# dcy0577/Enhancing-3D-Point-Cloud-Segmentation-Using-Multi-Modal-Fusion-with-2D-Images

Hardware: AMD Instinct MI355X
Metric: input points/s through MV-KPConv KPFCNN forward+backward (pyramid + fusion + fwd + bwd + SGD) (higher is better)
Workload: dtype f32; 1 GPU; early_fusion_kpfcnn5_sphere19k_x1_per_gpu; views=3, parallelism=dp1, execution=hipGraph[net|chain|enc2d(x2 every 2nd step)+fa], ranks=1, input_lookahead_batches=2, capacity_overflow=False

## Files before the change

### enhancing-3d-point-cloud-segmentation-using-multi-modal-fusion-with-2d-images_amd/_lib.py

```python
import ctypes as C
import os
import re

_HERE = os.path.dirname(os.path.abspath(__file__))
LIB_PATH = os.path.join(_HERE, "libmvkpconv.so")
HEADER_PATH = os.path.join(_HERE, "..", "include", "mvkpconv.h")
SCENE_HEADER_PATH = os.path.join(_HERE, "..", "include", "mvkpconv_scene.h")
TRAIN_HEADER_PATH = os.path.join(_HERE, "..", "include", "mvkpconv_train.h")
SPHERE_HEADER_PATH = os.path.join(_HERE, "..", "include", "mvkpconv_sphere.h")

CTYPES = {"int": C.c_int, "int32_t": C.c_int32, "int64_t": C.c_int64, "float": C.c_float, "double": C.c_double,
          "const char*": C.c_char_p}
_SCALARS = frozenset(t for t in CTYPES if not t.endswith("*"))
_POINTEES = _SCALARS | {"void", "char", "uint8_t", "uint16_t"}
_INTEGER = r"-?(?:0[xX][0-9a-fA-F]+|0|[1-9][0-9]*)"
_DIRECTIVE = re.compile(r"\s*#\s*(?:include\s*<[\w./]+>|ifdef\s+__cplusplus|ifndef\s+\w+_H|endif"
                        r"|define\s+(\w+)(?:\s+(%s))?)\s*" % _INTEGER)
_STRUCT = re.compile(r"typedef\s+struct(?:\s+\w+)?\s*\{([^{}]*)\}\s*(mvk_\w+)\s*;")
_FUNCTION = re.compile(r"([\w\s*]+?)\b(mvk_\w+)\s*\(([^(){};]*)\)\s*;")


def parse_header(text):
    functions, structs, constants = {}, {}, {}

# ... 101 lines not shown
    raise ValueError("mvkpconv_scene.h: it may declare neither a struct nor a name of mvkpconv.h")
_SCENE_PROTOTYPES = _bind(SCENE_FUNCTIONS, {})[1]

TRAIN_FUNCTIONS, _train_structs, TRAIN_CONSTANTS = parse_header(_read_header(TRAIN_HEADER_PATH, "mvkpconv_train.h"))
if (_train_structs or TRAIN_FUNCTIONS.keys() & (FUNCTIONS.keys() | SCENE_FUNCTIONS.keys())
        or TRAIN_CONSTANTS.keys() & (CONSTANTS.keys() | SCENE_CONSTANTS.keys())):
    raise ValueError("mvkpconv_train.h: it may declare neither a struct nor a name of the other two headers")
_TRAIN_PROTOTYPES = _bind(TRAIN_FUNCTIONS, {})[1]

SPHERE_FUNCTIONS, _sphere_structs, SPHERE_CONSTANTS = parse_header(_read_header(SPHERE_HEADER_PATH, "mvkpconv_sphere.h"))
if (_sphere_structs
        or SPHERE_FUNCTIONS.keys() & (FUNCTIONS.keys() | SCENE_FUNCTIONS.keys() | TRAIN_FUNCTIONS.keys())
        or SPHERE_CONSTANTS.keys() & (CONSTANTS.keys() | SCENE_CONSTANTS.keys() | TRAIN_CONSTANTS.keys())):
    raise ValueError("mvkpconv_sphere.h: it may declare neither a struct nor a name of the other three headers")
_SPHERE_PROTOTYPES = _bind(SPHERE_FUNCTIONS, {})[1]
BnFwdProblem, BnBwdProblem = _CLASSES["mvk_bn_fwd_problem"], _CLASSES["mvk_bn_bwd_problem"]
BnFinish, ATransform = _CLASSES["mvk_bn_finish"], _CLASSES["mvk_a_transform"]
RevList, RegLayer = _CLASSES["mvk_rev_list"], _CLASSES["mvk_reg_layer"]

_lib = None
_owner_pid = None

FORK_MESSAGE = ("the MV-KPConv HIP library was initialised in process %d and is being called from its forked child %d: "
                "a HIP context does not survive fork(). Start DataLoader workers with multiprocessing_context='spawn', "
                "or let the workers emit only stacked points / lengths and build the pyramid "
                "(datasets.common.segmentation_inputs_sphere) in the main process -- see INTEGRATION.md")


def _check_process():
    pid = os.getpid()
# ... 5 lines not shown
            raise RuntimeError(FORK_MESSAGE % (os.getppid(), pid))
    except (ImportError, AttributeError):
        pass


def lib():
    global _lib, _owner_pid
    _check_process()
    if _lib is None:
        if not os.path.exists(LIB_PATH):
            raise RuntimeError(
                "libmvkpconv.so is not built (%s). Run `python __graft_entry__.py build` -- there is "
                "no CPU fallback for the MV-KPConv hot path." % LIB_PATH)
        l = C.CDLL(LIB_PATH)
        for name, (res, args) in list(_PROTOTYPES.items()) + list(_SCENE_PROTOTYPES.items()) + list(_TRAIN_PROTOTYPES.items()) \
                + list(_SPHERE_PROTOTYPES.items()):
            fn = getattr(l, name)
            fn.restype = res
            fn.argtypes = args
        if l.mvk_abi_version() != ABI_VERSION:
            raise RuntimeError("libmvkpconv.so ABI %d != expected %d; rebuild" % (l.mvk_abi_version(), ABI_VERSION))
        _lib = l
        _owner_pid = os.getpid()
    return _lib


def check(rc):
    if rc != 0:
        raise RuntimeError(lib().mvk_last_error().decode("utf-8", "replace"))
```

### enhancing-3d-point-cloud-segmentation-using-multi-modal-fusion-with-2d-images_amd/build.py

```python
import os
import subprocess
import sys

HERE = os.path.dirname(os.path.abspath(__file__))
CSRC = os.path.join(HERE, "csrc")
OUT = os.path.join(HERE, "libmvkpconv.so")
ARCH = "gfx950"

SOURCES = [
    ("error.cpp", []),
    ("kpconv.hip", []),
    ("gemm.hip", []),
    ("gemm32s.hip", []),
    ("pool.hip", []),
    ("bn.hip", []),
    ("optim.hip", []),
    ("deform.hip", []),
    ("loss.hip", []),
    ("batchpad.hip", []),
    ("revlist.hip", []),
    ("subsample.hip", ["-ffp-contract=off"]),
    ("neighbors.hip", ["-ffp-contract=off"]),
    ("fusion.hip", ["-ffp-contract=off"]),
    ("vote.hip", ["-ffp-contract=off"]),
    ("pn2.hip", ["-ffp-contract=off"]),
    ("chunk.hip", ["-ffp-contract=off"]),
    ("pn2_ordered.hip", ["-ffp-contract=off"]),
    ("pn2_mlp.hip", ["-ffp-contract=off"]),
    ("pn2_rows.hip", ["-ffp-contract=off"]),
    ("scene_inputs.hip", ["-ffp-contract=off"]),
    ("train_inputs.hip", ["-ffp-contract=off"]),
    ("sphere_inputs.hip", ["-ffp-contract=off"]),
]
# ... 6 lines not shown
    return "hipcc"


def _stale(target, deps):
    if not os.path.exists(target):
        return True
    t = os.path.getmtime(target)
    return any(os.path.getmtime(d) > t for d in deps if os.path.exists(d))


def build_library(force=False, verbose=False):
    hipcc = _hipcc()
    common = [os.path.join(CSRC, "common.h"), os.path.join(CSRC, "blockscan.h"), os.path.join(CSRC, "compact.h"),
              os.path.join(CSRC, "pn2_rows.h"), os.path.join(CSRC, "unproject.h"), os.path.join(CSRC, "select_frames.h"),
              os.path.join(CSRC, "knn_core.h"), os.path.join(HERE, "..", "include", "mvkpconv_sphere.h"),
              os.path.join(HERE, "..", "include", "mvkpconv.h"), os.path.join(HERE, "..", "include", "mvkpconv_scene.h"),
              os.path.join(HERE, "..", "include", "mvkpconv_train.h"),
              os.path.join(HERE, "..", "include", "mvk_prime_list.h"), os.path.abspath(__file__)]
    objs, jobs = [], []
    for src, extra in SOURCES:
        sp = os.path.join(CSRC, src)
        if not os.path.exists(sp):
            raise FileNotFoundError(sp)
        obj = os.path.join(CSRC, os.path.splitext(src)[0] + ".o")
        if force or _stale(obj, [sp] + common):
            cmd = [hipcc, "--offload-arch=" + ARCH, "-O3", "-std=c++17", "-fPIC", "-c", sp, "-o", obj] + extra
            if src.endswith(".cpp"):
                cmd = [hipcc, "-O2", "-std=c++17", "-fPIC", "-c", sp, "-o", obj]
            jobs.append(cmd)
        objs.append(obj)
# ... 21 lines not shown
```

### enhancing-3d-point-cloud-segmentation-using-multi-modal-fusion-with-2d-images_amd/dropin/models/architectures.py

```python
import numpy as np
import torch
import torch.nn as nn

try:
    from .blocks import KPConv, UnaryBlock, NearestUpsampleBlock, block_decider
    from .._native import ops as _ops
except ImportError:
    from models.blocks import KPConv, UnaryBlock, NearestUpsampleBlock, block_decider
    from _native import ops as _ops


def p2p_fitting_regularizer(net):
    total = 0
    deform = [m for m in net.modules() if isinstance(m, KPConv) and m.deformable]
    if deform and all(m.min_d2.is_cuda for m in deform):
        term = _ops.deform_regularizer_all([(m.min_d2, m.deformed_KP, m.KP_extent, net.repulse_extent,
                                             net.deform_fitting_power, _ops.row_count_for(m.min_d2.shape[0]))
                                            for m in deform])
        return term if term is not None else total
    for m in deform:
        rows = m.min_d2.shape[0]
        n_valid = _ops.row_count_for(rows)
        if n_valid is None:
            mask, denom = None, float(rows)
# ... 85 lines not shown
        idx = labels.long().clamp(-1, lut.numel() - 2) + 1
        return lut[idx].to(labels.dtype)

    def _label_table(self, device, dtype=torch.int64):
        key = "_target_lut" if dtype == torch.int64 else "_target_lut32"
        lut = getattr(self, key, None)
        if lut is None or lut.device != device:
            top = int(max(self.valid_labels)) if len(self.valid_labels) else 0
            table = np.full(top + 3, -1, dtype=np.int64)
            for i, c in enumerate(self.valid_labels):
                table[int(c) + 1] = i
            lut = torch.from_numpy(table).to(device=device, dtype=dtype)
            setattr(self, key, lut)
        return lut

    def loss(self, outputs, labels):
        if outputs.is_cuda and outputs.dtype == torch.float32:
            self.output_loss = _ops.cross_entropy_lut(outputs, labels, self._label_table(outputs.device, torch.int32),
                                                      self.criterion.weight)
        else:
            target = self._targets(labels)
            outputs = torch.transpose(outputs, 0, 1).unsqueeze(0)
            self.output_loss = self.criterion(outputs, target.unsqueeze(0))
        if self.deform_fitting_mode == 'point2point':
            self.reg_loss = p2p_fitting_regularizer(self)
        elif self.deform_fitting_mode == 'point2plane':
            raise ValueError('point2plane fitting mode not implemented yet.')
        else:
            raise ValueError('Unknown fitting mode: ' + self.deform_fitting_mode)
        if isinstance(self.reg_loss, (int, float)) and self.reg_loss == 0:
            return self.output_loss
        return self.output_loss + self.reg_loss
# ... 56 lines not shown
    def __init__(self, config, lbl_values, ign_lbls):
        super(KPFCNN, self).__init__()
        self.K = config.num_kernel_points
        self.C = len(lbl_values) - len(ign_lbls)
        (self.encoder_blocks, self.encoder_skips, self.encoder_skip_dims,
         in_dim, out_dim, layer, r) = build_encoder(config, config.in_features_dim)
        self.decoder_blocks, self.decoder_concats, out_dim = build_decoder(
            config, in_dim, out_dim, layer, r, self.encoder_skip_dims)
        self.head_mlp = UnaryBlock(out_dim, config.first_features_dim, False, 0)
        self.head_softmax = UnaryBlock(config.first_features_dim, self.C, False, 0)
        self._init_losses(config, lbl_values, ign_lbls)

    def forward(self, batch, config):
        x = batch.features.detach()
        x = run_encoder_decoder(self, x, batch)
        return self.head_softmax(self.head_mlp(x, batch), batch)
```

### enhancing-3d-point-cloud-segmentation-using-multi-modal-fusion-with-2d-images_amd/dropin/models/architectures_sphere.py

```python
import torch
import torch.nn as nn

try:
    from .architectures import (p2p_fitting_regularizer, build_encoder, build_decoder, run_encoder_decoder,
                                _SegmentationLossMixin)
    from .blocks import UnaryBlock
    from .fusion_common import build_2d_branch, lift_2d_features
except ImportError:
    from models.architectures import (p2p_fitting_regularizer, build_encoder, build_decoder,
                                      run_encoder_decoder, _SegmentationLossMixin)
    from models.blocks import UnaryBlock
    from models.fusion_common import build_2d_branch, lift_2d_features


class KPFCNN_featureAggre(_SegmentationLossMixin, nn.Module):
    fa_output_detached = True

    def __init__(self, config, lbl_values, ign_lbls):
        super(KPFCNN_featureAggre, self).__init__()
        self.K = config.num_kernel_points
        self.C = len(lbl_values) - len(ign_lbls)
        (self.encoder_blocks, self.encoder_skips, self.encoder_skip_dims,
         in_dim, out_dim, layer, r) = build_encoder(config, config.in_features_dim)
        self.decoder_blocks, self.decoder_concats, out_dim = build_decoder(
            config, in_dim, out_dim, layer, r, self.encoder_skip_dims)
        self.head_mlp = UnaryBlock(out_dim, config.first_features_dim, False, 0)
        self.head_softmax = UnaryBlock(config.first_features_dim, self.C, False, 0)
        self._init_losses(config, lbl_values, ign_lbls)
        build_2d_branch(self, config)

    def forward(self, batch, config):
        stacked = getattr(batch, 'stacked_features', None)
        if stacked is None:
            feature_2d3d = lift_2d_features(self, batch)
            stacked = torch.cat((batch.feature_3d, feature_2d3d), dim=1)
        x = stacked.detach()
        x = run_encoder_decoder(self, x, batch)
        return self.head_softmax(self.head_mlp(x, batch), batch)
```

### enhancing-3d-point-cloud-segmentation-using-multi-modal-fusion-with-2d-images_amd/dropin/models/architectures_sphere_late_fusion.py

```python
import torch
import torch.nn as nn

try:
    from .architectures import (p2p_fitting_regularizer, build_encoder, build_decoder, run_encoder_decoder,
                                _SegmentationLossMixin)
    from .blocks import UnaryBlock
    from .fusion_common import build_2d_branch, lift_2d_features
except ImportError:
    from models.architectures import (p2p_fitting_regularizer, build_encoder, build_decoder,
                                      run_encoder_decoder, _SegmentationLossMixin)
    from models.blocks import UnaryBlock
    from models.fusion_common import build_2d_branch, lift_2d_features


class KPFCNN_featureAggre(_SegmentationLossMixin, nn.Module):

    def __init__(self, config, lbl_values, ign_lbls):
        super(KPFCNN_featureAggre, self).__init__()
        self.K = config.num_kernel_points
        self.C = len(lbl_values) - len(ign_lbls)
        (self.encoder_blocks, self.encoder_skips, self.encoder_skip_dims,
         in_dim, out_dim, layer, r) = build_encoder(config, config.in_features_dim)
        self.decoder_blocks, self.decoder_concats, out_dim = build_decoder(
            config, in_dim, out_dim, layer, r, self.encoder_skip_dims)
        self.transform_mlp = UnaryBlock(out_dim, 64, False, 0)
        self.head_mlp = UnaryBlock(out_dim, config.first_features_dim, False, 0)
        self.head_softmax = UnaryBlock(config.first_features_dim, self.C, False, 0)
        self._init_losses(config, lbl_values, ign_lbls)
        build_2d_branch(self, config)

    def forward(self, batch, config):
        feature_2d3d = lift_2d_features(self, batch)
        x = batch.feature_3d.detach()
        x = run_encoder_decoder(self, x, batch)
        x = self.transform_mlp(x, batch)
        x = torch.cat((x, feature_2d3d), dim=1)
        return self.head_softmax(self.head_mlp(x, batch), batch)
```

### enhancing-3d-point-cloud-segmentation-using-multi-modal-fusion-with-2d-images_amd/dropin/models/architectures_sphere_middle_fusion.py

```python
import torch
import torch.nn as nn

try:
    from .architectures import (p2p_fitting_regularizer, build_encoder, build_decoder, run_decoder,
                                _SegmentationLossMixin)
    from .blocks import UnaryBlock
    from .fusion_common import build_2d_branch, lift_2d_features
except ImportError:
    from models.architectures import (p2p_fitting_regularizer, build_encoder, build_decoder, run_decoder,
                                      _SegmentationLossMixin)
    from models.blocks import UnaryBlock
    from models.fusion_common import build_2d_branch, lift_2d_features


class KPFCNN_featureAggre(_SegmentationLossMixin, nn.Module):
    fa_output_detached = True

    def __init__(self, config, lbl_values, ign_lbls):
        super(KPFCNN_featureAggre, self).__init__()
        self.K = config.num_kernel_points
        self.C = len(lbl_values) - len(ign_lbls)
        (self.encoder_blocks_3d, self.encoder_skips, dims3, in3, out_dim, layer, r) = build_encoder(
            config, config.in_features_dim_3d)
        (self.encoder_blocks_2d, _, dims2, in2, _, _, _) = build_encoder(config, config.in_features_dim_2d)
# ... 11 lines not shown
        x_2d = torch.cat((ones, feature_2d3d), dim=1).detach()
        x_3d = batch.feature_3d.detach()
        skip_x = []
        for block_i, block_op in enumerate(self.encoder_blocks_3d):
            if block_i in self.encoder_skips:
                skip_x.append(x_3d)
            x_3d = block_op(x_3d, batch)
        index = 0
        for block_i, block_op in enumerate(self.encoder_blocks_2d):
            if block_i in self.encoder_skips:
                skip_x[index] = torch.cat([skip_x[index], x_2d], dim=1)
                index += 1
            x_2d = block_op(x_2d, batch)
        x = torch.mean(torch.stack([x_3d, x_2d]), 0)
        x = run_decoder(self, x, skip_x, batch)
        return self.head_softmax(self.head_mlp(x, batch), batch)
```

### enhancing-3d-point-cloud-segmentation-using-multi-modal-fusion-with-2d-images_amd/ops.py

```python
import collections
import os
import ctypes as C

import weakref

import torch

from ._lib import lib, check, CONSTANTS, SCENE_CONSTANTS, TRAIN_CONSTANTS, SPHERE_CONSTANTS

INFLUENCE = {k[len("MVK_INFL_"):].lower(): v for k, v in CONSTANTS.items() if k.startswith("MVK_INFL_")}
AGGREGATION = {k[len("MVK_AGG_"):].lower(): v for k, v in CONSTANTS.items() if k.startswith("MVK_AGG_")}


def _p(t):
    return C.c_void_p(t.data_ptr()) if t is not None else None


def _stream():
    return C.c_void_p(torch.cuda.current_stream().cuda_stream)


def _dev(*ts):
    for t in ts:
        if t is not None and not t.is_cuda:
# ... 2381 lines not shown
        d = torch.empty_like(logits)
        check(lib().mvk_xent_bwd(_p(logits), logits.shape[0], logits.shape[1], _p(labels),
                                 int(labels.dtype == torch.int64), _p(lut), lut.numel(), _p(weight), _p(out2), _p(g), _p(d),
                                 _stream()))
        return d, None, None, None


def cross_entropy_lut(logits, labels, lut, class_weight=None):
    if lut.dtype != torch.int32 or lut.dim() != 1 or lut.numel() < 3:
        raise RuntimeError("cross_entropy_lut: lut must be a 1-D int32 tensor of at least 3 entries")
    if logits.dim() != 2 or labels.dim() != 1 or labels.shape[0] != logits.shape[0]:
        raise RuntimeError("cross_entropy_lut: logits [N, C] and labels [N] expected")
    if class_weight is not None and (class_weight.dtype != torch.float32 or class_weight.numel() != logits.shape[1]):
        raise RuntimeError("cross_entropy_lut: class_weight must be float32 [C]")
    return _XentFn.apply(logits, labels, lut, None if class_weight is None else class_weight.contiguous())


_SEG_STATUS = {}


def seg_label_status(device):
    device = torch.device(device)
    key = device.index if device.index is not None else torch.cuda.current_device()
    if key not in _SEG_STATUS:
        _SEG_STATUS[key] = torch.zeros((1,), device=device, dtype=torch.int32)
    return _SEG_STATUS[key]


def seg_check_labels(device=None):
    status = seg_label_status(device if device is not None else torch.device("cuda", torch.cuda.current_device()))
# ... 781 lines not shown
```

### enhancing-3d-point-cloud-segmentation-using-multi-modal-fusion-with-2d-images_amd/step.py

```python
import os
import sys
import time

import numpy as np
import torch

from . import dp, ops, synthetic as syn

_DEV = {"on": False}
_DEV_KNOBS = ("MVK_BENCH_DIAG", "MVK_BENCH_SKIP", "MVK_BENCH_DUMMY_LAUNCHES")


def _knob(name, default=None):
    v = os.environ.get(name)
    if v is None or v == "":
        return default
    if not _DEV["on"]:
        raise RuntimeError("%s=%s is a development knob of the captured step (it changes what a step contains): pass "
                           "dev=True to GraphStep / --dev to bench.py, or unset it" % (name, v))
    return v


class GraphStep:

# ... 236 lines not shown
                else:
                    loss = torch.zeros((), device=dev)
                for h in hooks:
                    h.remove()
                if diag != "noside":
                    if not side_first and not hooks:
                        side_work()
                    join_encoder()
            return graph.replay, loss
        staged_exchange = hasattr(reducer, "cut_block")
        net.backward_cut = reducer.cut_block if staged_exchange else None
        scope = backward_scope(ops)
        with torch.cuda.graph(graph, stream=main_stream, capture_error_mode="thread_local"):
            hooks = fork_side_branches()
            ops.step_begin()
            loss = net.loss(net(static, cfg), static.labels)
            for h in hooks:
                h.remove()
            if staged_exchange:
                orig, leaves = net.cut_tensors
                with scope():
                    loss.backward(reducer.seed(loss), retain_graph=reducer.dp.deformable_below(cfg.architecture, reducer.cut_block))
                reducer.pack(0)
            else:
                backward(ops, loss)
            join_encoder()
        if not staged_exchange:
            graph_b = torch.cuda.CUDAGraph()
            with torch.cuda.graph(graph_b, stream=main_stream, pool=graph.pool(), capture_error_mode="thread_local"):
                clip_and_step(params, opt, cfg)
            grads = [p.grad for p in reducer.params if p.grad is not None]
# ... 229 lines not shown

def make_reducer(net, cfg, params, world):
    cut = dp.cut_block_of_layer(cfg.architecture, 2) if os.environ.get("MVK_DP_OVERLAP", "1") == "1" else None
    if cut is None or not hasattr(net, "encoder_blocks"):
        return dp.FlatAllReduce(params, world)
    late, early = dp.split_parameters_at(net, cut)
    comm = None
    if os.environ.get("MVK_DP_GRAPH_COLLECTIVES", "0") == "1" and torch.distributed.get_backend() == "nccl":
        comm = dp.RcclCommunicator(params[0].device)
    red = dp.BucketedAllReduce([late, early], world, comm=comm, prescaled=os.environ.get("MVK_DP_PRESCALE", "1") == "1")
    red.cut_block = cut
    red.dp = dp
    return red


def net_step_captured(net, static, cfg, params, opt, reducer, begin=True):
    if begin:
        ops.step_begin()
    staged_exchange = reducer is not None and hasattr(reducer, "cut_block")
    tail = split_tail_plan(net, cfg, opt) if reducer is None else None
    net.backward_cut = reducer.cut_block if staged_exchange else (tail["cut"] if tail else None)
    out = net(static, cfg)
    loss = net.loss(out, static.labels)
    if staged_exchange:
        def between():
            reducer.pack(0)
            reducer.launch(0)
        reducer.dp.two_stage_backward(loss, net.cut_tensors, between=between, backward_scope=backward_scope(ops),
                                      seed=reducer.seed(loss),
                                      retain_graph=reducer.dp.deformable_below(cfg.architecture, reducer.cut_block))
        reducer.pack(1)
        reducer.launch(1)
        reducer.wait()
        reducer.unpack(0)
        reducer.unpack(1)
    elif tail:
        split_tail_backward(ops, net, loss, opt, tail)
        return loss
# ... 72 lines not shown
```

Before: 5.438 million points/s.

## Fuse segmentation head MLP, LeakyReLU and cross-entropy into single forward/backward kernels

```diff
diff --git a/enhancing-3d-point-cloud-segmentation-using-multi-modal-fusion-with-2d-images_amd/_lib.py b/enhancing-3d-point-cloud-segmentation-using-multi-modal-fusion-with-2d-images_amd/_lib.py
--- a/enhancing-3d-point-cloud-segmentation-using-multi-modal-fusion-with-2d-images_amd/_lib.py
+++ b/enhancing-3d-point-cloud-segmentation-using-multi-modal-fusion-with-2d-images_amd/_lib.py
@@ -8,6 +8,7 @@
 SCENE_HEADER_PATH = os.path.join(_HERE, "..", "include", "mvkpconv_scene.h")
 TRAIN_HEADER_PATH = os.path.join(_HERE, "..", "include", "mvkpconv_train.h")
 SPHERE_HEADER_PATH = os.path.join(_HERE, "..", "include", "mvkpconv_sphere.h")
+HEAD_HEADER_PATH = os.path.join(_HERE, "..", "include", "mvkpconv_head.h")
 
 CTYPES = {"int": C.c_int, "int32_t": C.c_int32, "int64_t": C.c_int64, "float": C.c_float, "double": C.c_double,
           "const char*": C.c_char_p}
@@ -139,6 +140,13 @@
         or SPHERE_CONSTANTS.keys() & (CONSTANTS.keys() | SCENE_CONSTANTS.keys() | TRAIN_CONSTANTS.keys())):
     raise ValueError("mvkpconv_sphere.h: it may declare neither a struct nor a name of the other three headers")
 _SPHERE_PROTOTYPES = _bind(SPHERE_FUNCTIONS, {})[1]
+
+HEAD_FUNCTIONS, _head_structs, HEAD_CONSTANTS = parse_header(_read_header(HEAD_HEADER_PATH, "mvkpconv_head.h"))
+if (_head_structs
+        or HEAD_FUNCTIONS.keys() & (FUNCTIONS.keys() | SCENE_FUNCTIONS.keys() | TRAIN_FUNCTIONS.keys() | SPHERE_FUNCTIONS.keys())
+        or HEAD_CONSTANTS.keys() & (CONSTANTS.keys() | SCENE_CONSTANTS.keys() | TRAIN_CONSTANTS.keys() | SPHERE_CONSTANTS.keys())):
+    raise ValueError("mvkpconv_head.h: it may declare neither a struct nor a name of the other four headers")
+_HEAD_PROTOTYPES = _bind(HEAD_FUNCTIONS, {})[1]
 BnFwdProblem, BnBwdProblem = _CLASSES["mvk_bn_fwd_problem"], _CLASSES["mvk_bn_bwd_problem"]
 BnFinish, ATransform = _CLASSES["mvk_bn_finish"], _CLASSES["mvk_a_transform"]
 RevList, RegLayer = _CLASSES["mvk_rev_list"], _CLASSES["mvk_reg_layer"]
@@ -174,7 +182,7 @@
                 "no CPU fallback for the MV-KPConv hot path." % LIB_PATH)
         l = C.CDLL(LIB_PATH)
         for name, (res, args) in list(_PROTOTYPES.items()) + list(_SCENE_PROTOTYPES.items()) + list(_TRAIN_PROTOTYPES.items()) \
-                + list(_SPHERE_PROTOTYPES.items()):
+                + list(_SPHERE_PROTOTYPES.items()) + list(_HEAD_PROTOTYPES.items()):
             fn = getattr(l, name)
             fn.restype = res
             fn.argtypes = args
diff --git a/enhancing-3d-point-cloud-segmentation-using-multi-modal-fusion-with-2d-images_amd/build.py b/enhancing-3d-point-cloud-segmentation-using-multi-modal-fusion-with-2d-images_amd/build.py
--- a/enhancing-3d-point-cloud-segmentation-using-multi-modal-fusion-with-2d-images_amd/build.py
+++ b/enhancing-3d-point-cloud-segmentation-using-multi-modal-fusion-with-2d-images_amd/build.py
@@ -17,6 +17,7 @@
     ("optim.hip", []),
     ("deform.hip", []),
     ("loss.hip", []),
+    ("head.hip", []),
     ("batchpad.hip", []),
     ("revlist.hip", []),
     ("subsample.hip", ["-ffp-contract=off"]),
@@ -53,6 +54,7 @@
     common = [os.path.join(CSRC, "common.h"), os.path.join(CSRC, "blockscan.h"), os.path.join(CSRC, "compact.h"),
               os.path.join(CSRC, "pn2_rows.h"), os.path.join(CSRC, "unproject.h"), os.path.join(CSRC, "select_frames.h"),
               os.path.join(CSRC, "knn_core.h"), os.path.join(HERE, "..", "include", "mvkpconv_sphere.h"),
+              os.path.join(HERE, "..", "include", "mvkpconv_head.h"),
               os.path.join(HERE, "..", "include", "mvkpconv.h"), os.path.join(HERE, "..", "include", "mvkpconv_scene.h"),
               os.path.join(HERE, "..", "include", "mvkpconv_train.h"),
               os.path.join(HERE, "..", "include", "mvk_prime_list.h"), os.path.abspath(__file__)]
diff --git a/enhancing-3d-point-cloud-segmentation-using-multi-modal-fusion-with-2d-images_amd/csrc/head.hip b/enhancing-3d-point-cloud-segmentation-using-multi-modal-fusion-with-2d-images_amd/csrc/head.hip
--- /dev/null
+++ b/enhancing-3d-point-cloud-segmentation-using-multi-modal-fusion-with-2d-images_amd/csrc/head.hip
@@ -0,0 +1,494 @@
+#include "common.h"
+#include "../../include/mvkpconv_head.h"
+
+namespace {
+
+typedef float f4 __attribute__((ext_vector_type(4)));
+
+constexpr int TM = MVK_HEAD_TILE;
+constexpr int CMAX = MVK_HEAD_MAX_CLASSES;
+constexpr int CP = CMAX + 4;
+
+__device__ __forceinline__ f4 mfma4(f4 a, f4 b, f4 acc) {
+  acc = __builtin_amdgcn_mfma_f32_16x16x4f32(a.x, b.x, acc, 0, 0, 0);
+  acc = __builtin_amdgcn_mfma_f32_16x16x4f32(a.y, b.y, acc, 0, 0, 0);
+  acc = __builtin_amdgcn_mfma_f32_16x16x4f32(a.z, b.z, acc, 0, 0, 0);
+  acc = __builtin_amdgcn_mfma_f32_16x16x4f32(a.w, b.w, acc, 0, 0, 0);
+  return acc;
+}
+
+__device__ __forceinline__ float lrelu(float v, float slope) { return v > 0.f ? v : slope * v; }
+
+template <bool L64>
+__device__ __forceinline__ int class_of(const void* labels, int64_t i, const int32_t* __restrict__ lut, int lut_n) {
+  int64_t l = L64 ? ((const int64_t*)labels)[i] : (int64_t)((const int32_t*)labels)[i];
+  l = l < -1 ? -1 : (l > lut_n - 2 ? lut_n - 2 : l);
+  return lut[l + 1];
+}
+
+__device__ __forceinline__ float row_max(float v) {
+#pragma unroll
+  for (int o = 8; o > 0; o >>= 1) v = fmaxf(v, __shfl_xor(v, o));
+  return v;
+}
+__device__ __forceinline__ float row_sum(float v) {
+#pragma unroll
+  for (int o = 8; o > 0; o >>= 1) v += __shfl_xor(v, o);
+  return v;
+}
+
+__device__ __forceinline__ void tile_out(const float* __restrict__ tile, int S, float* __restrict__ out, int64_t row0,
+                                         int64_t N, int W) {
+  const int q = W >> 2;
+  for (int i = threadIdx.x; i < TM * q; i += 256) {
+    const int row = i / q, c4 = i - row * q;
+    if (row0 + row < N) *(f4*)(out + (row0 + row) * W + 4 * c4) = *(const f4*)(tile + row * S + 4 * c4);
+  }
+}
+
+constexpr int KS = 4;
+constexpr int WS = 16 * KS + 4;
+
+template <int NT>
+__device__ __forceinline__ void product_kk(const float* a, const float* const (&b)[NT], int K, f4 (&acc)[NT]) {
+  for (int k0 = 0; k0 < K; k0 += 16 * KS) {
+    f4 av[KS], bv[KS][NT];
+#pragma unroll
+    for (int s = 0; s < KS; ++s) {
+      const bool in = k0 + 16 * s < K;
+      const int k = in ? k0 + 16 * s : k0;
+      av[s] = *(const f4*)(a + k);
+#pragma unroll
+      for (int u = 0; u < NT; ++u) bv[s][u] = *(const f4*)(b[u] + k);
+    }
+    __builtin_amdgcn_sched_barrier(0);
+#pragma unroll
+    for (int s = 0; s < KS; ++s) {
+      const f4 as = k0 + 16 * s < K ? av[s] : (f4){0.f, 0.f, 0.f, 0.f};
+#pragma unroll
+      for (int u = 0; u < NT; ++u) acc[u] = mfma4(as, bv[s][u], acc[u]);
+    }
+  }
+}
+
+template <int NT>
+__device__ __forceinline__ void product_kn(const float* a, const float* __restrict__ b, int ldb, int K, f4 (&acc)[NT]) {
+  for (int k0 = 0; k0 < K; k0 += 16 * KS) {
+    f4 av[KS], bv[KS][NT];
+#pragma unroll
+    for (int s = 0; s < KS; ++s) {
+      const bool in = k0 + 16 * s < K;
+      const int k = in ? k0 + 16 * s : k0;
+      av[s] = *(const f4*)(a + k);
+      const float* bk = b + (int64_t)k * ldb;
+#pragma unroll
+      for (int u = 0; u < NT; ++u) bv[s][u] = (f4){bk[u * 16], bk[ldb + u * 16], bk[2 * ldb + u * 16], bk[3 * ldb + u * 16]};
+    }
+    __builtin_amdgcn_sched_barrier(0);
+#pragma unroll
+    for (int s = 0; s < KS; ++s) {
+      const f4 as = k0 + 16 * s < K ? av[s] : (f4){0.f, 0.f, 0.f, 0.f};
+#pragma unroll
+      for (int u = 0; u < NT; ++u) acc[u] = mfma4(as, bv[s][u], acc[u]);
+    }
+  }
+}
+
+template <bool L64, int NT>
+__global__ __launch_bounds__(256) void head_fwd_k(const float* __restrict__ x, int64_t N, int K1,
+                                                  const float* __restrict__ W1, const float* __restrict__ b1, float s1,
+                                                  int Hd, const float* __restrict__ W2, const float* __restrict__ b2,
+                                                  float s2, int C, const void* labels, const int32_t* __restrict__ lut,
+                                                  int lut_n, const float* __restrict__ weight, float* __restrict__ h,
+                                                  float* __restrict__ logits, float* __restrict__ partials) {
+  extern __shared__ float hs[];
+  __shared__ float rl[TM], rw[TM];
+  const int lane = threadIdx.x & 63, w = threadIdx.x >> 6, c = lane & 15, g = lane >> 4;
+  const int HS = Hd + 4, HT = Hd >> 4;
+  const int64_t row0 = (int64_t)blockIdx.x * TM;
+  const int64_t ar = row0 + 16 * w + c;
+  const float* xa = x + (ar < N ? ar : N - 1) * K1 + 4 * g;
+  int tcls[4];
+  float wcls[4];
+#pragma unroll
+  for (int r = 0; r < 4; ++r) {
+    const int64_t gr = row0 + 16 * w + 4 * g + r;
+    const int t = labels && gr < N ? class_of<L64>(labels, gr, lut, lut_n) : -1;
+    tcls[r] = t >= 0 && t < C ? t : -1;
+    wcls[r] = tcls[r] < 0 ? 0.f : (weight ? weight[t] : 1.f);
+  }
+
+  float* ws = hs + TM * HS;
+  for (int ct0 = 0; ct0 < HT; ct0 += NT) {
+    f4 acc[NT];
+#pragma unroll
+    for (int u = 0; u < NT; ++u) acc[u] = (f4){0.f, 0.f, 0.f, 0.f};
+    const float* wg = W1 + (int64_t)ct0 * 16 * K1;
+    f4 wr[NT];
+#pragma unroll
+    for (int i = 0; i < NT; ++i) {
+      const int row = (threadIdx.x >> 4) + 16 * i, k = 4 * (threadIdx.x & 15);
+      wr[i] = *(const f4*)(wg + (int64_t)row * K1 + (k < K1 ? k : 0));
+    }
+    f4 av[KS];
+#pragma unroll
+    for (int s = 0; s < KS; ++s) av[s] = *(const f4*)(xa + (16 * s < K1 ? 16 * s : 0));
+    for (int k0 = 0; k0 < K1; k0 += 16 * KS) {
+      __syncthreads();
+#pragma unroll
+      for (int i = 0; i < NT; ++i) *(f4*)(ws + ((threadIdx.x >> 4) + 16 * i) * WS + 4 * (threadIdx.x & 15)) = wr[i];
+      __syncthreads();
+      const int kn = k0 + 16 * KS < K1 ? k0 + 16 * KS : k0;
+#pragma unroll
+      for (int i = 0; i < NT; ++i) {
+        const int row = (threadIdx.x >> 4) + 16 * i, k = kn + 4 * (threadIdx.x & 15);
+        wr[i] = *(const f4*)(wg + (int64_t)row * K1 + (k < K1 ? k : kn));
+      }
+      f4 an[KS];
+#pragma unroll
+      for (int s = 0; s < KS; ++s) an[s] = *(const f4*)(xa + (kn + 16 * s < K1 ? kn + 16 * s : kn));
+      f4 bf[2][NT];
+#pragma unroll
+      for (int u = 0; u < NT; ++u) bf[0][u] = *(const f4*)(ws + (16 * u + c) * WS + 4 * g);
+      __builtin_amdgcn_sched_barrier(0);
+#pragma unroll
+      for (int s = 0; s < KS; ++s) {
+        if (s + 1 < KS) {
+#pragma unroll
+          for (int u = 0; u < NT; ++u) bf[(s + 1) & 1][u] = *(const f4*)(ws + (16 * u + c) * WS + 16 * (s + 1) + 4 * g);
+        }
+        __builtin_amdgcn_sched_barrier(0);
+        const f4 as = k0 + 16 * s < K1 ? av[s] : (f4){0.f, 0.f, 0.f, 0.f};
+#pragma unroll
+        for (int u = 0; u < NT; ++u) acc[u] = mfma4(as, bf[s & 1][u], acc[u]);
+        __builtin_amdgcn_sched_barrier(0);
+      }
+#pragma unroll
+      for (int s = 0; s < KS; ++s) av[s] = an[s];
+    }
+#pragma unroll
+    for (int u = 0; u < NT; ++u) {
+      const int col = (ct0 + u) * 16 + c;
+      const float bias = b1[col];
+#pragma unroll
+      for (int r = 0; r < 4; ++r) hs[(16 * w + 4 * g + r) * HS + col] = lrelu(acc[u][r] + bias, s1);
+    }
+  }
+  __syncthreads();
+  tile_out(hs, HS, h, row0, N, Hd);
+
+  const int n0 = c, n1 = 16 + c;
+  const bool in0 = n0 < C, in1 = n1 < C;
+  const float* ha = hs + (16 * w + c) * HS + 4 * g;
+  const float* const w2[2] = {W2 + (int64_t)(in0 ? n0 : C - 1) * Hd + 4 * g, W2 + (int64_t)(in1 ? n1 : C - 1) * Hd + 4 * g};
+  f4 lg2[2] = {{0.f, 0.f, 0.f, 0.f}, {0.f, 0.f, 0.f, 0.f}};
+  product_kk<2>(ha, w2, Hd, lg2);
+  const f4 l0 = lg2[0], l1 = lg2[1];
+  const float bias0 = b2[in0 ? n0 : C - 1], bias1 = b2[in1 ? n1 : C - 1];
+#pragma unroll
+  for (int r = 0; r < 4; ++r) {
+    const int row = 16 * w + 4 * g + r;
+    const int64_t gr = row0 + row;
+    const bool live = gr < N;
+    const float v0 = lrelu(l0[r] + bias0, s2), v1 = lrelu(l1[r] + bias1, s2);
+    if (live && in0) logits[gr * C + n0] = v0;
+    if (live && in1) logits[gr * C + n1] = v1;
+    if (labels) {
+      const int t = tcls[r];
+      const bool kept = t >= 0;
+      const float m = row_max(fmaxf(in0 ? v0 : -INFINITY, in1 ? v1 : -INFINITY));
+      const float s = row_sum((in0 ? expf(v0 - m) : 0.f) + (in1 ? expf(v1 - m) : 0.f));
+      const float xt = row_sum((n0 == t ? v0 : 0.f) + (n1 == t ? v1 : 0.f));
+      if (c == 0) {
+        const float wi = wcls[r];
+        rw[row] = wi;
+        rl[row] = kept ? wi * (logf(s) + m - xt) : 0.f;
+      }
+    }
+  }
+  if (!labels) return;
+  __syncthreads();
+  if (w == 0) {
+    float a = rl[lane], b = rw[lane];
+#pragma unroll
+    for (int o = 32; o > 0; o >>= 1) {
+      a += __shfl_xor(a, o);
+      b += __shfl_xor(b, o);
+    }
+    if (lane == 0) {
+      partials[2 * blockIdx.x] = a;
+      partials[2 * blockIdx.x + 1] = b;
+    }
+  }
+}
+
+__global__ __launch_bounds__(64) void head_loss_finish_k(const float* __restrict__ partials, int nblk,
+                                                         float* __restrict__ out2) {
+  __shared__ float sa[64], sb[64];
+  float a = 0.f, b = 0.f;
+  for (int g = threadIdx.x; g < nblk; g += 64) {
+    a += partials[2 * g];
+    b += partials[2 * g + 1];
+  }
+  sa[threadIdx.x] = a;
+  sb[threadIdx.x] = b;
+  __syncthreads();
+  if (threadIdx.x == 0) {
+    a = 0.f;
+    b = 0.f;
+    for (int l = 0; l < 64; ++l) {
+      a += sa[l];
+      b += sb[l];
+    }
+    out2[0] = a / b;
+    out2[1] = b;
+  }
+}
+
+template <bool L64, int NT>
+__global__ __launch_bounds__(256) void head_bwd_k(int64_t N, int K1, const float* __restrict__ W1, float s1, int Hd,
+                                                  const float* __restrict__ W2, float s2, int C,
+                                                  const float* __restrict__ h, const float* __restrict__ logits,
+                                                  const void* labels, const int32_t* __restrict__ lut, int lut_n,
+                                                  const float* __restrict__ weight, const float* __restrict__ out2,
+                                                  const float* __restrict__ gl, const float* __restrict__ g_logits,
+                                                  float* __restrict__ dz2, float* __restrict__ dz1,
+                                                  float* __restrict__ dx, float* __restrict__ pb, int ntiles) {
+  extern __shared__ float d1s[];
+  __shared__ float lg[TM * CMAX];
+  __shared__ float d2s[TM * CP];
+  const int tid = threadIdx.x, lane = tid & 63, w = tid >> 6, c = lane & 15, g = lane >> 4;
+  const int HS = Hd + 4, HT = Hd >> 4, KT = K1 >> 4;
+  const int64_t row0 = (int64_t)blockIdx.x * TM;
+  const int rows = (int)(N - row0 < TM ? N - row0 : TM);
+
+  int t = -1;
+  float kf = 0.f;
+  if (labels) {
+    if ((tid >> 2) < rows) t = class_of<L64>(labels, row0 + (tid >> 2), lut, lut_n);
+    if (t >= C) t = -1;
+    if (t >= 0) kf = gl[0] * (weight ? weight[t] : 1.f) / out2[1];
+  }
+  for (int i = tid; i < rows * C; i += 256) lg[i] = logits[row0 * C + i];
+  __syncthreads();
+
+  if (labels) {
+    const int row = tid >> 2, q = tid & 3;
+    const float* r = lg + row * C;
+    const bool kept = t >= 0;
+    float m = -INFINITY, s = 0.f;
+    if (kept)
+      for (int k = q; k < C; k += 4) m = fmaxf(m, r[k]);
+    m = fmaxf(m, __shfl_xor(m, 1));
+    m = fmaxf(m, __shfl_xor(m, 2));
+    if (kept)
+      for (int k = q; k < C; k += 4) s += expf(r[k] - m);
+    s += __shfl_xor(s, 1);
+    s += __shfl_xor(s, 2);
+    const float inv = 1.f / s;
+    for (int k = q; k < CMAX; k += 4) {
+      float v = 0.f;
+      if (kept && k < C) v = kf * (expf(r[k] - m) * inv - (k == t ? 1.f : 0.f)) * (r[k] > 0.f ? 1.f : s2);
+      d2s[row * CP + k] = v;
+    }
+  } else {
+    for (int i = tid; i < TM * CMAX; i += 256) {
+      const int row = i >> 5, k = i & 31;
+      float v = 0.f;
+      if (row < rows && k < C) v = g_logits[(row0 + row) * C + k] * (lg[row * C + k] > 0.f ? 1.f : s2);
+      d2s[row * CP + k] = v;
+    }
+  }
+  __syncthreads();
+
+  for (int i = tid; i < rows * C; i += 256) {
+    const int row = i / C;
+    dz2[row0 * C + i] = d2s[row * CP + (i - row * C)];
+  }
+  if (tid < C) {
+    float s = 0.f;
+    for (int row = 0; row < TM; ++row) s += d2s[row * CP + tid];
+    pb[(int64_t)tid * ntiles + blockIdx.x] = s;
+  }
+
+  const int KC = (C + 3) & ~3;
+  const float* d2a = d2s + (16 * w + c) * CP;
+  for (int ct0 = 0; ct0 < HT; ct0 += NT) {
+    f4 acc[NT];
+#pragma unroll
+    for (int u = 0; u < NT; ++u) acc[u] = (f4){0.f, 0.f, 0.f, 0.f};
+    const float* wc = W2 + ct0 * 16 + c;
+    for (int k0 = 0; k0 < KC; k0 += 4 * KS) {
+      float av[KS], bv[KS][NT];
+#pragma unroll
+      for (int s = 0; s < KS; ++s) {
+        const int k = k0 + 4 * s + g;
+        av[s] = d2a[k];
+        const float* wr = wc + (int64_t)(k < C ? k : C - 1) * Hd;
+#pragma unroll
+        for (int u = 0; u < NT; ++u) bv[s][u] = wr[u * 16];
+      }
+      __builtin_amdgcn_sched_barrier(0);
+#pragma unroll
+      for (int s = 0; s < KS; ++s)
+#pragma unroll
+        for (int u = 0; u < NT; ++u) acc[u] = __builtin_amdgcn_mfma_f32_16x16x4f32(av[s], bv[s][u], acc[u], 0, 0, 0);
+    }
+#pragma unroll
+    for (int u = 0; u < NT; ++u) {
+      const int col = (ct0 + u) * 16 + c;
+#pragma unroll
+      for (int r = 0; r < 4; ++r) {
+        const int row = 16 * w + 4 * g + r;
+        const float hv = h[(row0 + (row < rows ? row : rows - 1)) * Hd + col];
+        d1s[row * HS + col] = acc[u][r] * (hv > 0.f ? 1.f : s1);
+      }
+    }
+  }
+  __syncthreads();
+  tile_out(d1s, HS, dz1, row0, N, Hd);
+  if (tid < Hd) {
+    float s = 0.f;
+    for (int row = 0; row < TM; ++row) s += d1s[row * HS + tid];
+    pb[(int64_t)(C + tid) * ntiles + blockIdx.x] = s;
+  }
+  if (!dx) return;
+
+  const float* da = d1s + (16 * w + c) * HS + 4 * g;
+  for (int ct0 = 0; ct0 < KT; ct0 += NT) {
+    f4 acc[NT];
+#pragma unroll
+    for (int u = 0; u < NT; ++u) acc[u] = (f4){0.f, 0.f, 0.f, 0.f};
+    product_kn<NT>(da, W1 + (int64_t)(4 * g) * K1 + ct0 * 16 + c, K1, Hd, acc);
+#pragma unroll
+    for (int u = 0; u < NT; ++u) {
+      const int col = (ct0 + u) * 16 + c;
+#pragma unroll
+      for (int r = 0; r < 4; ++r) {
+        const int row = 16 * w + 4 * g + r;
+        if (row < rows) dx[(row0 + row) * K1 + col] = acc[u][r];
+      }
+    }
+  }
+}
+
+__global__ __launch_bounds__(256) void head_bias_finish_k(const float* __restrict__ pb, int ntiles, int C, int Hd,
+                                                          float* __restrict__ db2, float* __restrict__ db1) {
+  const int lane = threadIdx.x & 63, col = blockIdx.x * 4 + (threadIdx.x >> 6);
+  if (col >= C + Hd) return;
+  const float* p = pb + (int64_t)col * ntiles;
+  float s = 0.f;
+  for (int t = lane; t < ntiles; t += 64) s += p[t];
+#pragma unroll
+  for (int o = 32; o > 0; o >>= 1) s += __shfl_xor(s, o);
+  if (lane == 0) (col < C ? db2[col] : db1[col - C]) = s;
+}
+
+int head_sizes(int64_t N, int K1, int Hd, int C) {
+  MVK_REQUIRE(N >= 0 && N < (1LL << 31), "head: N=%lld rows, 0 <= N < 2^31 expected", (long long)N);
+  MVK_REQUIRE(K1 >= 16 && K1 <= MVK_HEAD_MAX_WIDTH && K1 % 16 == 0 && Hd >= 16 && Hd <= MVK_HEAD_MAX_WIDTH && Hd % 16 == 0,
+              "head: K1=%d and Hd=%d must be multiples of 16 in [16, %d]", K1, Hd, MVK_HEAD_MAX_WIDTH);
+  MVK_REQUIRE(C >= 1 && C <= MVK_HEAD_MAX_CLASSES, "head: C=%d classes, 1 <= C <= %d expected", C, MVK_HEAD_MAX_CLASSES);
+  return 0;
+}
+
+bool aligned16(const void* p) { return ((uintptr_t)p & 15) == 0; }
+
+template <typename K>
+int head_lds(K kernel, int Hd, int extra, size_t* bytes) {
+  static size_t granted[64] = {};
+  *bytes = sizeof(float) * (TM * (Hd + 4) + extra);
+  if (*bytes <= 40 * 1024) return 0;
+  int dev = 0;
+  MVK_CHECK_HIP(hipGetDevice(&dev));
+  if (dev < 0 || dev >= 64 || granted[dev] < *bytes) {
+    MVK_CHECK_HIP(hipFuncSetAttribute((const void*)kernel, hipFuncAttributeMaxDynamicSharedMemorySize, (int)*bytes));
+    if (dev >= 0 && dev < 64) granted[dev] = *bytes;
+  }
+  return 0;
+}
+
+int tiles_at_once(int a, int b) {
+  for (int nt = 8; nt > 1; nt >>= 1)
+    if (a % nt == 0 && b % nt == 0) return nt;
+  return 1;
+}
+
+template <bool L64, int NT, typename... A>
+int fwd_launch(unsigned gx, int Hd, hipStream_t st, A... a) {
+  size_t lds;
+  if (int rc = head_lds(head_fwd_k<L64, NT>, Hd, NT * 16 * WS, &lds)) return rc;
+  hipLaunchKernelGGL((head_fwd_k<L64, NT>), dim3(gx), dim3(256), lds, st, a...);
+  return 0;
+}
+
+template <bool L64, int NT, typename... A>
+int bwd_launch(unsigned gx, int Hd, hipStream_t st, A... a) {
+  size_t lds;
+  if (int rc = head_lds(head_bwd_k<L64, NT>, Hd, 0, &lds)) return rc;
+  hipLaunchKernelGGL((head_bwd_k<L64, NT>), dim3(gx), dim3(256), lds, st, a...);
+  return 0;
+}
+
+#define HEAD_PICK(launch, l64, nt, ...)                                                        \
+  ((nt) == 8   ? ((l64) ? launch<true, 8>(__VA_ARGS__) : launch<false, 8>(__VA_ARGS__))         \
+   : (nt) == 4 ? ((l64) ? launch<true, 4>(__VA_ARGS__) : launch<false, 4>(__VA_ARGS__))         \
+   : (nt) == 2 ? ((l64) ? launch<true, 2>(__VA_ARGS__) : launch<false, 2>(__VA_ARGS__))         \
+               : ((l64) ? launch<true, 1>(__VA_ARGS__) : launch<false, 1>(__VA_ARGS__)))
+
+}
+
+extern "C" int mvk_head_workspace(int64_t N, int K1, int Hd, int C, int64_t* loss_floats_host, int64_t* bias_floats_host,
+                                  void* stream) {
+  (void)stream;
+  if (int rc = head_sizes(N, K1, Hd, C)) return rc;
+  MVK_REQUIRE(loss_floats_host && bias_floats_host, "head: null operand");
+  const int64_t tiles = cdiv64(N > 0 ? N : 1, TM);
+  *loss_floats_host = 2 * tiles;
+  *bias_floats_host = tiles * (C + Hd);
+  return 0;
+}
+
+extern "C" int mvk_head_fwd(const float* x, int64_t N, int K1, const float* W1, const float* b1, float slope1, int Hd,
+                            const float* W2, const float* b2, float slope2, int C, const void* labels, int labels64,
+                            const int32_t* lut, int lut_n, const float* class_weight, float* h, float* logits,
+                            float* partials, float* out2, void* stream) {
+  if (int rc = head_sizes(N, K1, Hd, C)) return rc;
+  MVK_REQUIRE(slope1 > 0.f && slope2 > 0.f, "head: both slopes must be positive (%g, %g)", slope1, slope2);
+  if (N == 0) return 0;
+  MVK_REQUIRE(x && W1 && b1 && W2 && b2 && h && logits, "head: null operand");
+  MVK_REQUIRE(!labels || (lut && lut_n >= 3 && partials && out2), "head: labels need lut (>= 3 entries), partials and out2");
+  MVK_REQUIRE(aligned16(x) && aligned16(W1) && aligned16(W2) && aligned16(h), "head: x, W1, W2 and h must be 16-byte aligned");
+  hipStream_t st = (hipStream_t)stream;
+  const unsigned gx = (unsigned)cdiv64(N, TM);
+  if (int rc = HEAD_PICK(fwd_launch, labels64 != 0, tiles_at_once(Hd / 16, Hd / 16), gx, Hd, st, x, N, K1, W1, b1, slope1, Hd, W2, b2,
+                         slope2, C, labels, lut, lut_n, class_weight, h, logits, partials))
+    return rc;
+  if (labels) hipLaunchKernelGGL(head_loss_finish_k, dim3(1), dim3(64), 0, st, partials, (int)gx, out2);
+  MVK_CHECK_HIP(hipGetLastError());
+  return 0;
+}
+
+extern "C" int mvk_head_bwd(int64_t N, int K1, const float* W1, float slope1, int Hd, const float* W2, float slope2, int C,
+                            const float* h, const float* logits, const void* labels, int labels64, const int32_t* lut,
+                            int lut_n, const float* class_weight, const float* out2, const float* grad_loss,
+                            const float* g_logits, float* dz2, float* dz1, float* dx, float* bias_partials, float* db2,
+                            float* db1, void* stream) {
+  if (int rc = head_sizes(N, K1, Hd, C)) return rc;
+  MVK_REQUIRE(slope1 > 0.f && slope2 > 0.f, "head: both slopes must be positive (%g, %g)", slope1, slope2);
+  if (N == 0) return 0;
+  MVK_REQUIRE(W1 && W2 && h && logits && dz2 && dz1 && bias_partials && db2 && db1, "head: null operand");
+  MVK_REQUIRE(labels ? (lut && lut_n >= 3 && out2 && grad_loss) : g_logits != nullptr,
+              "head: the backward needs labels with lut (>= 3 entries), out2 and grad_loss, or g_logits");
+  MVK_REQUIRE(aligned16(dz1), "head: dz1 must be 16-byte aligned");
+  hipStream_t st = (hipStream_t)stream;
+  const unsigned gx = (unsigned)cdiv64(N, TM);
+  if (int rc = HEAD_PICK(bwd_launch, labels64 != 0, tiles_at_once(Hd / 16, K1 / 16), gx, Hd, st, N, K1, W1, slope1, Hd, W2, slope2,
+                         C, h, logits, labels, lut, lut_n, class_weight, out2, grad_loss, g_logits, dz2, dz1, dx, bias_partials,
+                         (int)gx))
+    return rc;
+  hipLaunchKernelGGL(head_bias_finish_k, dim3((unsigned)cdiv64(C + Hd, 4)), dim3(256), 0, st, bias_partials, (int)gx, C, Hd, db2,
+                     db1);
+  MVK_CHECK_HIP(hipGetLastError());
+  return 0;
+}
diff --git a/enhancing-3d-point-cloud-segmentation-using-multi-modal-fusion-with-2d-images_amd/dropin/models/architectures.py b/enhancing-3d-point-cloud-segmentation-using-multi-modal-fusion-with-2d-images_amd/dropin/models/architectures.py
--- a/enhancing-3d-point-cloud-segmentation-using-multi-modal-fusion-with-2d-images_amd/dropin/models/architectures.py
+++ b/enhancing-3d-point-cloud-segmentation-using-multi-modal-fusion-with-2d-images_amd/dropin/models/architectures.py
@@ -123,8 +123,29 @@
             setattr(self, key, lut)
         return lut
 
+    def head(self, x, batch):
+        m1, m2 = self.head_mlp, self.head_softmax
+        if not (_ops.HEAD_FUSED and x.is_cuda and x.dim() == 2 and self.training and torch.is_grad_enabled()
+                and not m1.use_bn and not m2.use_bn):
+            return m2(m1(x, batch), batch)
+        args = (x, m1.mlp.weight, m1.batch_norm.bias, 1.0 if m1.no_relu else 0.1,
+                m2.mlp.weight, m2.batch_norm.bias, 1.0 if m2.no_relu else 0.1)
+        labels = getattr(self, "loss_labels", None)
+        if labels is None:
+            return _ops.head(*args)
+        logits, loss = _ops.head_xent(*args, labels, self._label_table(x.device, torch.int32), self.criterion.weight)
+        logits._mvk_head_loss = (loss, labels)
+        return logits
+
     def loss(self, outputs, labels):
-        if outputs.is_cuda and outputs.dtype == torch.float32:
+        handed = getattr(outputs, "_mvk_head_loss", None)
+        if handed is not None and handed[1] is not labels and not outputs.requires_grad:
+            raise RuntimeError("loss(): these logits were computed together with the loss of the labels handed over "
+                               "before the forward (net.loss_labels) and carry no graph of their own; pass that "
+                               "very tensor, or run the forward without the hand-over")
+        if handed is not None and handed[1] is labels:
+            self.output_loss = handed[0]
+        elif outputs.is_cuda and outputs.dtype == torch.float32:
             self.output_loss = _ops.cross_entropy_lut(outputs, labels, self._label_table(outputs.device, torch.int32),
                                                       self.criterion.weight)
         else:
@@ -211,4 +232,4 @@
     def forward(self, batch, config):
         x = batch.features.detach()
         x = run_encoder_decoder(self, x, batch)
-        return self.head_softmax(self.head_mlp(x, batch), batch)
+        return self.head(x, batch)
diff --git a/enhancing-3d-point-cloud-segmentation-using-multi-modal-fusion-with-2d-images_amd/dropin/models/architectures_sphere.py b/enhancing-3d-point-cloud-segmentation-using-multi-modal-fusion-with-2d-images_amd/dropin/models/architectures_sphere.py
--- a/enhancing-3d-point-cloud-segmentation-using-multi-modal-fusion-with-2d-images_amd/dropin/models/architectures_sphere.py
+++ b/enhancing-3d-point-cloud-segmentation-using-multi-modal-fusion-with-2d-images_amd/dropin/models/architectures_sphere.py
@@ -36,4 +36,4 @@
             stacked = torch.cat((batch.feature_3d, feature_2d3d), dim=1)
         x = stacked.detach()
         x = run_encoder_decoder(self, x, batch)
-        return self.head_softmax(self.head_mlp(x, batch), batch)
+        return self.head(x, batch)
diff --git a/enhancing-3d-point-cloud-segmentation-using-multi-modal-fusion-with-2d-images_amd/dropin/models/architectures_sphere_late_fusion.py b/enhancing-3d-point-cloud-segmentation-using-multi-modal-fusion-with-2d-images_amd/dropin/models/architectures_sphere_late_fusion.py
--- a/enhancing-3d-point-cloud-segmentation-using-multi-modal-fusion-with-2d-images_amd/dropin/models/architectures_sphere_late_fusion.py
+++ b/enhancing-3d-point-cloud-segmentation-using-multi-modal-fusion-with-2d-images_amd/dropin/models/architectures_sphere_late_fusion.py
@@ -35,4 +35,4 @@
         x = run_encoder_decoder(self, x, batch)
         x = self.transform_mlp(x, batch)
         x = torch.cat((x, feature_2d3d), dim=1)
-        return self.head_softmax(self.head_mlp(x, batch), batch)
+        return self.head(x, batch)
diff --git a/enhancing-3d-point-cloud-segmentation-using-multi-modal-fusion-with-2d-images_amd/dropin/models/architectures_sphere_middle_fusion.py b/enhancing-3d-point-cloud-segmentation-using-multi-modal-fusion-with-2d-images_amd/dropin/models/architectures_sphere_middle_fusion.py
--- a/enhancing-3d-point-cloud-segmentation-using-multi-modal-fusion-with-2d-images_amd/dropin/models/architectures_sphere_middle_fusion.py
+++ b/enhancing-3d-point-cloud-segmentation-using-multi-modal-fusion-with-2d-images_amd/dropin/models/architectures_sphere_middle_fusion.py
@@ -49,4 +49,4 @@
             x_2d = block_op(x_2d, batch)
         x = torch.mean(torch.stack([x_3d, x_2d]), 0)
         x = run_decoder(self, x, skip_x, batch)
-        return self.head_softmax(self.head_mlp(x, batch), batch)
+        return self.head(x, batch)
diff --git a/enhancing-3d-point-cloud-segmentation-using-multi-modal-fusion-with-2d-images_amd/ops.py b/enhancing-3d-point-cloud-segmentation-using-multi-modal-fusion-with-2d-images_amd/ops.py
--- a/enhancing-3d-point-cloud-segmentation-using-multi-modal-fusion-with-2d-images_amd/ops.py
+++ b/enhancing-3d-point-cloud-segmentation-using-multi-modal-fusion-with-2d-images_amd/ops.py
@@ -6,7 +6,7 @@
 
 import torch
 
-from ._lib import lib, check, CONSTANTS, SCENE_CONSTANTS, TRAIN_CONSTANTS, SPHERE_CONSTANTS
+from ._lib import lib, check, CONSTANTS, SCENE_CONSTANTS, TRAIN_CONSTANTS, SPHERE_CONSTANTS, HEAD_CONSTANTS
 
 INFLUENCE = {k[len("MVK_INFL_"):].lower(): v for k, v in CONSTANTS.items() if k.startswith("MVK_INFL_")}
 AGGREGATION = {k[len("MVK_AGG_"):].lower(): v for k, v in CONSTANTS.items() if k.startswith("MVK_AGG_")}
@@ -2419,6 +2419,107 @@
     if class_weight is not None and (class_weight.dtype != torch.float32 or class_weight.numel() != logits.shape[1]):
         raise RuntimeError("cross_entropy_lut: class_weight must be float32 [C]")
     return _XentFn.apply(logits, labels, lut, None if class_weight is None else class_weight.contiguous())
+
+
+HEAD_FUSED = os.environ.get("MVK_HEAD_FUSED", "1") == "1"
+
+
+def _head_workspace(N, K1, Hd, Cc):
+    loss_floats, bias_floats = C.c_int64(), C.c_int64()
+    check(lib().mvk_head_workspace(N, K1, Hd, Cc, C.byref(loss_floats), C.byref(bias_floats), None))
+    return loss_floats.value, bias_floats.value
+
+
+def head_fused_supported(x, W1, b1, s1, W2, b2, s2):
+    ts = (x, W1, b1, W2, b2)
+    if not all(t.is_cuda and t.dtype == torch.float32 and t.is_contiguous() and t.data_ptr() % 16 == 0 for t in ts):
+        return False
+    if x.dim() != 2 or W1.dim() != 2 or W2.dim() != 2 or b1.dim() != 1 or b2.dim() != 1 or x.shape[0] == 0:
+        return False
+    (Hd, K1), (Cc, Hd2), width = W1.shape, W2.shape, HEAD_CONSTANTS["MVK_HEAD_MAX_WIDTH"]
+    return (x.shape[1] == K1 and Hd2 == Hd and b1.shape[0] == Hd and b2.shape[0] == Cc and s1 > 0 and s2 > 0
+            and K1 % 16 == 0 and Hd % 16 == 0 and 16 <= K1 <= width and 16 <= Hd <= width
+            and 1 <= Cc <= HEAD_CONSTANTS["MVK_HEAD_MAX_CLASSES"] and x.shape[0] < 2 ** 31)
+
+
+class _HeadFn(torch.autograd.Function):
+
+    @staticmethod
+    def forward(ctx, x, W1, b1, W2, b2, s1, s2, labels, lut, weight):
+        N, K1 = x.shape
+        Hd, Cc = W1.shape[0], W2.shape[0]
+        h = torch.empty((N, Hd), device=x.device, dtype=torch.float32)
+        logits = torch.empty((N, Cc), device=x.device, dtype=torch.float32)
+        part = out2 = None
+        if labels is not None:
+            part = torch.empty((_head_workspace(N, K1, Hd, Cc)[0],), device=x.device, dtype=torch.float32)
+            out2 = torch.empty((2,), device=x.device, dtype=torch.float32)
+        check(lib().mvk_head_fwd(_p(x), N, K1, _p(W1), _p(b1), s1, Hd, _p(W2), _p(b2), s2, Cc, _p(labels),
+                                 int(labels is not None and labels.dtype == torch.int64), _p(lut),
+                                 0 if lut is None else lut.numel(), _p(weight), _p(h), _p(logits), _p(part), _p(out2),
+                                 _stream()))
+        ctx.save_for_backward(x, W1, W2, h, logits, labels, lut, weight, out2)
+        ctx.slopes = (s1, s2)
+        if labels is None:
+            return logits
+        ctx.mark_non_differentiable(logits)
+        ctx.set_materialize_grads(False)
+        return logits, out2[0]
+
+    @staticmethod
+    def backward(ctx, g_logits, g_loss=None):
+        x, W1, W2, h, logits, labels, lut, weight, out2 = ctx.saved_tensors
+        (N, K1), Hd, Cc = x.shape, W1.shape[0], W2.shape[0]
+        if labels is not None and g_loss is None:
+            return (None,) * 10
+        g = _f32c(g_logits if labels is None else g_loss)
+        dz2, dz1 = torch.empty_like(logits), torch.empty_like(h)
+        dx = torch.empty_like(x) if ctx.needs_input_grad[0] else None
+        pb = torch.empty((_head_workspace(N, K1, Hd, Cc)[1],), device=x.device, dtype=torch.float32)
+        db1 = torch.empty((Hd,), device=x.device, dtype=torch.float32)
+        db2 = torch.empty((Cc,), device=x.device, dtype=torch.float32)
+        check(lib().mvk_head_bwd(N, K1, _p(W1), ctx.slopes[0], Hd, _p(W2), ctx.slopes[1], Cc, _p(h), _p(logits), _p(labels),
+                                 int(labels is not None and labels.dtype == torch.int64), _p(lut),
+                                 0 if lut is None else lut.numel(), _p(weight), _p(out2),
+                                 None if labels is None else _p(g), _p(g) if labels is None else None,
+                                 _p(dz2), _p(dz1), _p(dx), _p(pb), _p(db2), _p(db1), _stream()))
+        dW2 = _dw_gemm(dz2, h, target=W2) if ctx.needs_input_grad[3] else None
+        dW1 = _dw_gemm(dz1, x, target=W1) if ctx.needs_input_grad[1] else None
+        return dx, dW1, db1, dW2, db2, None, None, None, None, None
+
+
+def _head_operands(x, W1, b1, s1, W2, b2, s2):
+    _dev(x, W1, b1, W2, b2)
+    if not (s1 > 0 and s2 > 0):
+        raise ValueError("head: both slopes must be positive")
+    return _f32c(x), _f32c(W1), _f32c(b1), float(s1), _f32c(W2), _f32c(b2), float(s2)
+
+
+def head(x, W1, b1, s1, W2, b2, s2):
+    ops_ = _head_operands(x, W1, b1, s1, W2, b2, s2)
+    if HEAD_FUSED and head_fused_supported(*ops_):
+        x, W1, b1, s1, W2, b2, s2 = ops_
+        return _HeadFn.apply(x, W1, b1, W2, b2, s1, s2, None, None, None)
+    return linear_bias_lrelu(linear_bias_lrelu(x, W1, b1, s1), W2, b2, s2)
+
+
+def head_xent(x, W1, b1, s1, W2, b2, s2, labels, lut, class_weight=None):
+    if lut.dtype != torch.int32 or lut.dim() != 1 or lut.numel() < 3:
+        raise RuntimeError("head_xent: lut must be a 1-D int32 tensor of at least 3 entries")
+    if labels.dim() != 1 or labels.shape[0] != x.shape[0]:
+        raise RuntimeError("head_xent: labels [N] expected")
+    if class_weight is not None and (class_weight.dtype != torch.float32 or class_weight.numel() != W2.shape[0]):
+        raise RuntimeError("head_xent: class_weight must be float32 [C]")
+    ops_ = _head_operands(x, W1, b1, s1, W2, b2, s2)
+    if HEAD_FUSED and head_fused_supported(*ops_):
+        _dev(labels, lut, class_weight)
+        if labels.dtype not in (torch.int32, torch.int64):
+            labels = labels.long()
+        x, W1, b1, s1, W2, b2, s2 = ops_
+        return _HeadFn.apply(x, W1, b1, W2, b2, s1, s2, labels.contiguous(), lut.contiguous(),
+                             None if class_weight is None else class_weight.contiguous())
+    logits = linear_bias_lrelu(linear_bias_lrelu(x, W1, b1, s1), W2, b2, s2)
+    return logits, cross_entropy_lut(logits, labels, lut, class_weight)
 
 
 _SEG_STATUS = {}
diff --git a/enhancing-3d-point-cloud-segmentation-using-multi-modal-fusion-with-2d-images_amd/step.py b/enhancing-3d-point-cloud-segmentation-using-multi-modal-fusion-with-2d-images_amd/step.py
--- a/enhancing-3d-point-cloud-segmentation-using-multi-modal-fusion-with-2d-images_amd/step.py
+++ b/enhancing-3d-point-cloud-segmentation-using-multi-modal-fusion-with-2d-images_amd/step.py
@@ -274,7 +274,7 @@
         with torch.cuda.graph(graph, stream=main_stream, capture_error_mode="thread_local"):
             hooks = fork_side_branches()
             ops.step_begin()
-            loss = net.loss(net(static, cfg), static.labels)
+            loss = forward_and_loss(net, static, cfg)
             for h in hooks:
                 h.remove()
             if staged_exchange:
@@ -534,14 +534,22 @@
     return red
 
 
+def forward_and_loss(net, static, cfg):
+    net.loss_labels = static.labels
+    try:
+        out = net(static, cfg)
+    finally:
+        net.loss_labels = None
+    return net.loss(out, static.labels)
+
+
 def net_step_captured(net, static, cfg, params, opt, reducer, begin=True):
     if begin:
         ops.step_begin()
     staged_exchange = reducer is not None and hasattr(reducer, "cut_block")
     tail = split_tail_plan(net, cfg, opt) if reducer is None else None
     net.backward_cut = reducer.cut_block if staged_exchange else (tail["cut"] if tail else None)
-    out = net(static, cfg)
-    loss = net.loss(out, static.labels)
+    loss = forward_and_loss(net, static, cfg)
     if staged_exchange:
         def between():
             reducer.pack(0)
diff --git a/include/mvkpconv_head.h b/include/mvkpconv_head.h
--- /dev/null
+++ b/include/mvkpconv_head.h
@@ -0,0 +1,30 @@
+#ifndef MVKPCONV_HEAD_H
+#define MVKPCONV_HEAD_H
+
+#include <stdint.h>
+
+#ifdef __cplusplus
+extern "C" {
+#endif
+
+#define MVK_HEAD_TILE 64
+#define MVK_HEAD_MAX_WIDTH 256
+#define MVK_HEAD_MAX_CLASSES 32
+
+int mvk_head_workspace(int64_t N, int K1, int Hd, int C, int64_t* loss_floats_host, int64_t* bias_floats_host,
+                       void* stream);
+
+int mvk_head_fwd(const float* x, int64_t N, int K1, const float* W1, const float* b1, float slope1, int Hd,
+                 const float* W2, const float* b2, float slope2, int C, const void* labels, int labels64,
+                 const int32_t* lut, int lut_n, const float* class_weight, float* h, float* logits, float* partials,
+                 float* out2, void* stream);
+
+int mvk_head_bwd(int64_t N, int K1, const float* W1, float slope1, int Hd, const float* W2, float slope2, int C,
+                 const float* h, const float* logits, const void* labels, int labels64, const int32_t* lut, int lut_n,
+                 const float* class_weight, const float* out2, const float* grad_loss, const float* g_logits,
+                 float* dz2, float* dz1, float* dx, float* bias_partials, float* db2, float* db1, void* stream);
+
+#ifdef __cplusplus
+}
+#endif
+#endif
```

Result: faster. 5.494 million points/s, median of 6 (+1.0%).
